# dcharatan/flowmap

Hardware: NVIDIA H100
Metric: overfit iters/sec at 150x360x640 (149 frame pairs per iteration) (higher is better)
Workload: dtype f32

## Files before the change

### flowmap_b200/csrc/fm_kernels.cu

```cuda
#include <cuda_runtime.h>
#include <stdio.h>
#include <string.h>
#include <stdlib.h>

#include "../../include/flowmap_b200.h"
#include "fm_ate.cuh"
#include "fm_host.h"
#include "fm_pixel.cuh"

namespace fm_host {
namespace {
thread_local char g_err[512] = "";
unsigned long long g_launches = 0;
}
int fail(const char* what, cudaError_t e) {
  snprintf(g_err, sizeof(g_err), "%s: %s", what, cudaGetErrorString(e));
  return 1;
}
int fail_msg(const char* what) {
  snprintf(g_err, sizeof(g_err), "%s", what);
  return 2;
}
void count_launch() { __atomic_add_fetch(&g_launches, 1, __ATOMIC_RELAXED); }
const char* last_error() { return g_err; }
// ... 1409 lines not shown
    p[i] = pp; m[i] = mm; v[i] = vv;
  }
}

__global__ void __launch_bounds__(kThreads)
k_adam_frames_ragged(float* __restrict__ p, const float* __restrict__ g, float* __restrict__ m, float* __restrict__ v,
                     size_t frame_elems, const int* __restrict__ row_offset, int pairs, int lo, int hi, float beta1,
                     float beta2, float omb1, float omb2, float eps, const float* __restrict__ consts) {
  const float step_size = __ldg(consts), bc2_sqrt = __ldg(consts + 1);
  const int span = hi - lo, b = blockIdx.y / span, f = lo + (blockIdx.y - b * span);
  const int r0 = __ldg(row_offset + b);
  if (f >= __ldg(row_offset + b + 1) - r0 - pairs) return;
  const size_t o = ((size_t)(r0 - pairs * b) + f) * frame_elems;
  p += o; g += o; m += o; v += o;
  for (size_t i = (size_t)blockIdx.x * kThreads + threadIdx.x; i < frame_elems; i += (size_t)gridDim.x * kThreads) {
    float pp = p[i], gg = g[i], mm = m[i], vv = v[i];
    FM_ADAM1(pp, gg, mm, vv)
    p[i] = pp; m[i] = mm; v[i] = vv;
  }
#undef FM_ADAM1
}

constexpr int kTrackAcc = 10;
constexpr int kTrackRec = 24;

struct SegInfo { int sample_start, rows, n, start_frame; };

struct TrackShard {
  int depth_frame0, src_lo, src_hi;
  __device__ __forceinline__ bool owns(int frame) const { return frame >= src_lo && frame < src_hi; }
};

__device__ __forceinline__ SegInfo load_seg(const int* seg, int s) {
  const int4 v = __ldg(reinterpret_cast<const int4*>(seg) + s);
  SegInfo i; i.sample_start = v.x; i.rows = v.y; i.n = v.z; i.start_frame = v.w;
  return i;
}

__device__ __forceinline__ void load_segment_frames(float* sm, const float* ext, const float* k4,
                                                    const SegInfo& si, int source_frame) {
  const float* Ps = ext + (size_t)source_frame * 16;
  for (int row = threadIdx.x; row < si.rows; row += blockDim.x) {
    const float* P = ext + (size_t)(si.start_frame + row) * 16;
    float* o = sm + row * kTrackRec;
    float v[kTrackRec];
    float* R = v;
    double t[3];
#pragma unroll
    for (int i = 0; i < 3; ++i) {
      R[i * 3 + 0] = __ldg(P + i * 4 + 0); R[i * 3 + 1] = __ldg(P + i * 4 + 1); R[i * 3 + 2] = __ldg(P + i * 4 + 2);
      t[i] = (double)__ldg(P + i * 4 + 3) - (double)__ldg(Ps + i * 4 + 3);
      v[9 + i] = (float)t[i];
    }
#pragma unroll
    for (int i = 0; i < 3; ++i)
      v[12 + i] = (float)-((double)R[0 * 3 + i] * t[0] + (double)R[1 * 3 + i] * t[1] + (double)R[2 * 3 + i] * t[2]);
    const float4 k = __ldg(reinterpret_cast<const float4*>(k4) + si.start_frame + row);
    v[15] = k.x; v[16] = k.y; v[17] = k.z; v[18] = k.w; v[19] = 1.0f / k.x; v[20] = 1.0f / k.y;
    v[21] = v[22] = v[23] = 0.f;
#pragma unroll
    for (int i = 0; i < kTrackRec / 4; ++i)
      reinterpret_cast<float4*>(o)[i] = make_float4(v[4 * i], v[4 * i + 1], v[4 * i + 2], v[4 * i + 3]);
  }
  __syncthreads();
}
static_assert(kTrackRec % 4 == 0, "frame records are read as float4");
struct TrackRec {
  float R[9], t[3], c[3];
  Cam k;
};
__device__ __forceinline__ TrackRec load_rec(const float* rec) {
  const float4* r4 = reinterpret_cast<const float4*>(rec);
  const float4 a = r4[0], b = r4[1], c = r4[2], d = r4[3], e = r4[4], f = r4[5];
  TrackRec r;
  r.R[0] = a.x; r.R[1] = a.y; r.R[2] = a.z; r.R[3] = a.w; r.R[4] = b.x; r.R[5] = b.y; r.R[6] = b.z; r.R[7] = b.w;
  r.R[8] = c.x; r.t[0] = c.y; r.t[1] = c.z; r.t[2] = c.w;
  r.c[0] = d.x; r.c[1] = d.y; r.c[2] = d.z;
  r.k.fx = d.w; r.k.fy = e.x; r.k.cx = e.y; r.k.cy = e.z; r.k.ifx = e.w; r.k.ify = f.x;
  return r;
}

struct TrackSlot { int slot; bool owner; };
template <int N, int OFF>
struct SlotWalk {
  __device__ __forceinline__ static void run(int lane, int& pos, bool& ok) {
    if (N == 1) {
      SlotWalk<1, OFF / 2>::run(lane, pos, ok);
      ok = ok && (lane & OFF) == 0;
    } else {
      constexpr int HALF = (N + 1) / 2;
      SlotWalk<HALF, OFF / 2>::run(lane, pos, ok);
      if (lane & OFF) pos += HALF;
      ok = ok && pos < N;
    }
  }
};
template <int N>
struct SlotWalk<N, 0> {
  __device__ __forceinline__ static void run(int, int& pos, bool& ok) { pos = 0; ok = true; }
};
template <int N>
__device__ __forceinline__ TrackSlot track_slot(int lane) {
  TrackSlot t;
  SlotWalk<N, 16>::run(lane, t.slot, t.owner);
  return t;
}
template <int N, int OFF>
__device__ __forceinline__ void halve_exchange(float* v, bool upper) {
  constexpr int HALF = (N + 1) / 2;
#pragma unroll
  for (int j = 0; j < HALF; ++j) {
    const float hi = (j + HALF < N) ? v[j + HALF] : 0.f;
    const float send = upper ? v[j] : hi;
    const float keep = upper ? hi : v[j];
    v[j] = keep + __shfl_xor_sync(0xffffffffu, send, OFF);
  }
}
template <int N, int OFF>
struct WarpSumN {
  __device__ __forceinline__ static void run(float* v, int lane) {
    if (N == 1) {
      v[0] += __shfl_xor_sync(0xffffffffu, v[0], OFF);
      WarpSumN<1, OFF / 2>::run(v, lane);
    } else {
      halve_exchange<N, OFF>(v, lane & OFF);
      WarpSumN<(N + 1) / 2, OFF / 2>::run(v, lane);
    }
  }
};
template <int N>
struct WarpSumN<N, 0> {
  __device__ __forceinline__ static void run(float*, int) {}
};
template <int N>
__device__ __forceinline__ float warp_sum_n(float* v, int lane) {
  WarpSumN<N, 16>::run(v, lane);
  return v[0];
}

constexpr int kTrackThreads = 128;
#ifndef FM_TRACK_PPT
#define FM_TRACK_PPT 2
#endif
#ifndef FM_TRACK_BPS
#define FM_TRACK_BPS 5
#endif
#ifndef FM_TRACK_PARTS
#define FM_TRACK_PARTS 2
#endif
constexpr int kTrackParts = FM_TRACK_PARTS;
constexpr int kTrackPPT = FM_TRACK_PPT;
constexpr int kTrackPass = 32 * kTrackPPT;
constexpr int kTrackListCap = 2048;
static_assert(kTrackPPT == 1 || kTrackPPT == 2, "FM_TRACK_PPT must be 1 or 2");

__host__ __device__ constexpr size_t track_smem_bytes(int max_rows, int list_cap) {
  return ((size_t)max_rows * (kTrackRec + (kTrackThreads / 32) * kTrackAcc) + (size_t)list_cap) * sizeof(float);
}

struct TrackOneVideo {
  static constexpr bool kPerFrameK = true;
  using Scale = Uniform::Scale;
  template <class T> __device__ __forceinline__ T* sums_of(T* sums, int) const { return sums; }
};
struct TrackVideos {
  static constexpr bool kPerFrameK = false;
  using Scale = Videos::Scale;
  const int* frame_video;
  template <class T>
  __device__ __forceinline__ T* sums_of(T* sums, int f) const { return sums + 2 * __ldg(frame_video + f); }
};

template <bool SHARED_K, class TL>
__global__ void __launch_bounds__(kTrackThreads, FM_TRACK_BPS)
k_track_src(const float* __restrict__ depth, const float* __restrict__ k4, const float* __restrict__ ext,
            const int* __restrict__ seg, const float* __restrict__ txy, const unsigned char* __restrict__ tvis,
            int mapping, float delta, double* __restrict__ sums, unsigned char* __restrict__ flag,
            float* __restrict__ dq_out, double* __restrict__ trackacc, int* __restrict__ next_item, int num_items,
            int max_rows, int list_cap, int H, int W, TrackShard sh, TL tl) {
  extern __shared__ float4 sm4[];
  __shared__ double red[kTrackAcc * (kTrackThreads / 32)];
  __shared__ int s_wbase[kTrackThreads / 32];
  __shared__ int s_item[2];
  float* sm = reinterpret_cast<float*>(sm4);
  constexpr int NW = kTrackThreads / 32;
  constexpr int NRED = SHARED_K ? 6 : kTrackAcc;
  constexpr int SLOT0 = kTrackAcc - NRED;
  float* s_tgt = sm + (size_t)max_rows * kTrackRec;
  int* s_list = reinterpret_cast<int*>(s_tgt + (size_t)NW * max_rows * kTrackAcc);
  const GridDims grid = make_grid(H, W);
  const RobustCfg rc = make_robust(mapping, delta, H, W);
  const int lane = threadIdx.x & 31, warp = threadIdx.x >> 5;
  const TrackSlot slot = track_slot<NRED>(lane);
  const float2* xy2 = reinterpret_cast<const float2*>(txy);
  for (int it = 0;; ++it) {
    if (threadIdx.x == 0) s_item[it & 1] = atomicAdd(next_item, 1);
    __syncthreads();
    const int item = s_item[it & 1];
    if (item >= num_items) break;
    const int part = item % kTrackParts, srow = item / kTrackParts;
    const SegInfo si = load_seg(seg, srow / max_rows);
    const int row = srow % max_rows;
    if (row >= si.rows || !sh.owns(si.start_frame + row)) continue;
    load_segment_frames(sm, ext, k4, si, si.start_frame + row);
    float* tgt = s_tgt + (size_t)warp * si.rows * kTrackAcc;
    for (int i = lane; i < si.rows * kTrackAcc; i += 32) tgt[i] = 0.f;
    __syncwarp();
    const int frame = si.start_frame + row;
    const float* D = depth + (size_t)(frame - sh.depth_frame0) * H * W;
    const float* rsrec = sm + row * kTrackRec;
    const size_t row0 = (size_t)si.sample_start + (size_t)row * si.n;
    const float2* seg_xy = xy2 + si.sample_start;
    const unsigned char* seg_vis = tvis + si.sample_start;
    float acc[kTrackAcc], lc[2] = {0.f, 0.f};
#pragma unroll
    for (int i = 0; i < kTrackAcc; ++i) acc[i] = 0.f;
    const int p_end = (int)((long long)si.n * (part + 1) / kTrackParts);
    for (int base = (int)((long long)si.n * part / kTrackParts); base < p_end; base += list_cap) {
      const int len = min(list_cap, p_end - base);
      const int per = (len + NW * 32 - 1) / (NW * 32) * 32;
      const int lo = base + warp * per, hi = min(base + len, lo + per);
      int cnt = 0;
      for (int p0 = lo; p0 < hi; p0 += 32) {
        const int p = p0 + lane;
        bool ok = false;
        if (p < hi) {
          const size_t sidx = row0 + p;
          const float2 sxy = __ldg(xy2 + sidx);
          ok = tvis[sidx] && in_unit_square(sxy.x, sxy.y);
          flag[sidx] = ok ? 1 : 0;
        }
        cnt += __popc(__ballot_sync(0xffffffffu, ok));
      }
      if (lane == 0) s_wbase[warp] = cnt;
      __syncthreads();
      int wb = 0, total = 0;
#pragma unroll
      for (int w = 0; w < NW; ++w) {
        const int c = s_wbase[w];
        if (w < warp) wb += c;
        total += c;
      }
      for (int p0 = lo; p0 < hi; p0 += 32) {
        const int p = p0 + lane;
        const bool ok = p < hi && flag[row0 + p];
        const unsigned m = __ballot_sync(0xffffffffu, ok);
        if (ok) s_list[wb + __popc(m & ((1u << lane) - 1u))] = p;
        wb += __popc(m);
      }
      __syncthreads();
      const int npass = (total + kTrackPass - 1) / kTrackPass;
      for (int ps = warp; ps < npass; ps += NW) {
        const int pb = ps * kTrackPass + lane;
        float Xw[kTrackPPT][3];
        int ix[kTrackPPT];
        {
          const TrackRec rs = load_rec(rsrec);
#pragma unroll
          for (int j = 0; j < kTrackPPT; ++j) {
            Xw[j][0] = Xw[j][1] = Xw[j][2] = 0.f;
            ix[j] = -1;
            if (pb + 32 * j < total) {
              const int p = s_list[pb + 32 * j];
              ix[j] = p;
              const float2 sxy = __ldg(xy2 + row0 + p);
              const Taps t = bilinear_taps(sxy.x, sxy.y, grid);
              float q[3];
              sample_surface(t, grid, rs.k, [D](int o) { return __ldg(D + o); }, q[0], q[1], q[2]);
#pragma unroll
              for (int i = 0; i < 3; ++i)
                Xw[j][i] = fm_fma(rs.R[i * 3 + 0], q[0], fm_fma(rs.R[i * 3 + 1], q[1], fm_fma(rs.R[i * 3 + 2], q[2], rs.t[i])));
            }
          }
        }
        float G[kTrackPPT][3];
#pragma unroll
        for (int j = 0; j < kTrackPPT; ++j) G[j][0] = G[j][1] = G[j][2] = 0.f;
        unsigned char vn[kTrackPPT];
        float2 gn[kTrackPPT];
#pragma unroll
        for (int j = 0; j < kTrackPPT; ++j) {
          vn[j] = ix[j] >= 0 ? seg_vis[ix[j]] : 0;
          gn[j] = ix[j] >= 0 ? __ldg(seg_xy + ix[j]) : make_float2(0.f, 0.f);
        }
        for (int ft = 0; ft < si.rows; ++ft) {
          unsigned char v[kTrackPPT];
          float2 g[kTrackPPT];
          bool any = false;
#pragma unroll
          for (int j = 0; j < kTrackPPT; ++j) {
            v[j] = vn[j]; g[j] = gn[j];
            any |= v[j] != 0;
            if (ft + 1 < si.rows && ix[j] >= 0) {
              ix[j] += si.n;
              vn[j] = seg_vis[ix[j]];
              gn[j] = __ldg(seg_xy + ix[j]);
            }
          }
          float c[NRED];
#pragma unroll
          for (int i = 0; i < NRED; ++i) c[i] = 0.f;
          bool ok = false;
          if (any) {
            const TrackRec r = load_rec(sm + ft * kTrackRec);
#pragma unroll
            for (int j = 0; j < kTrackPPT; ++j) {
              const float dir0 = fm_fma(r.R[0], Xw[j][0], fm_fma(r.R[3], Xw[j][1], __fmul_rn(r.R[6], Xw[j][2])));
              const float dir1 = fm_fma(r.R[1], Xw[j][0], fm_fma(r.R[4], Xw[j][1], __fmul_rn(r.R[7], Xw[j][2])));
              const float dir2 = fm_fma(r.R[2], Xw[j][0], fm_fma(r.R[5], Xw[j][1], __fmul_rn(r.R[8], Xw[j][2])));
              const LeanTerm lt = lean_term(1.0f, dir0, dir1, dir2, r.c[0], r.c[1], r.c[2], r.k, g[j].x, g[j].y, 0.f,
                                            0.f, 1.0f, rc);
              const bool o = v[j] && in_unit_square(lt.uvx, lt.uvy);
              ok |= o;
              const float d0 = o ? lt.d0 : 0.f, d1 = o ? lt.d1 : 0.f, d2 = o ? lt.d2 : 0.f;
              lc[0] = __fadd_rn(lc[0], o ? lt.loss : 0.f);
              lc[1] = __fadd_rn(lc[1], o ? 1.f : 0.f);
              const float g0 = fm_fma(r.R[0], d0, fm_fma(r.R[1], d1, __fmul_rn(r.R[2], d2)));
              const float g1 = fm_fma(r.R[3], d0, fm_fma(r.R[4], d1, __fmul_rn(r.R[5], d2)));
              const float g2 = fm_fma(r.R[6], d0, fm_fma(r.R[7], d1, __fmul_rn(r.R[8], d2)));
              G[j][0] = __fadd_rn(G[j][0], g0); G[j][1] = __fadd_rn(G[j][1], g1); G[j][2] = __fadd_rn(G[j][2], g2);
              const float ex = __fmul_rn(d0, r.k.ifx), ey = __fmul_rn(d1, r.k.ify);
              if (SHARED_K) {
                acc[0] = fm_fma(ex, lt.P0, acc[0]); acc[1] = fm_fma(ey, lt.P1, acc[1]);
                acc[2] = fm_fma(ex, lt.P2, acc[2]); acc[3] = fm_fma(ey, lt.P2, acc[3]);
              } else {
                c[0] = __fadd_rn(c[0], __fmul_rn(ex, lt.P0)); c[1] = __fadd_rn(c[1], __fmul_rn(ey, lt.P1));
                c[2] = __fadd_rn(c[2], __fmul_rn(ex, lt.P2)); c[3] = __fadd_rn(c[3], __fmul_rn(ey, lt.P2));
              }
              const float e0 = __fsub_rn(Xw[j][0], r.t[0]), e1 = __fsub_rn(Xw[j][1], r.t[1]);
              const float e2 = __fsub_rn(Xw[j][2], r.t[2]);
              float* tw = c + (SHARED_K ? 0 : 4);
              tw[0] = __fadd_rn(tw[0], fm_fma(e2, g1, -__fmul_rn(e1, g2)));
              tw[1] = __fadd_rn(tw[1], fm_fma(e0, g2, -__fmul_rn(e2, g0)));
              tw[2] = __fadd_rn(tw[2], fm_fma(e1, g0, -__fmul_rn(e0, g1)));
              tw[3] = __fsub_rn(tw[3], g0); tw[4] = __fsub_rn(tw[4], g1); tw[5] = __fsub_rn(tw[5], g2);
            }
          }
          if (__ballot_sync(0xffffffffu, ok)) {
            const float total_c = warp_sum_n<NRED>(c, lane);
            if (slot.owner) tgt[ft * kTrackAcc + SLOT0 + slot.slot] += total_c;
          }
        }
        const TrackRec rs = load_rec(rsrec);
#pragma unroll
        for (int j = 0; j < kTrackPPT; ++j) {
          if (pb + 32 * j >= total) continue;
          const size_t sidx = row0 + s_list[pb + 32 * j];
          const float2 sxy = __ldg(xy2 + sidx);
          const Taps t = bilinear_taps(sxy.x, sxy.y, grid);
          float q[3];
          sample_surface(t, grid, rs.k, [D](int o) { return __ldg(D + o); }, q[0], q[1], q[2]);
          const float G0 = G[j][0], G1 = G[j][1], G2 = G[j][2];
          const float dq0 = fm_fma(rs.R[0], G0, fm_fma(rs.R[3], G1, rs.R[6] * G2));
          const float dq1 = fm_fma(rs.R[1], G0, fm_fma(rs.R[4], G1, rs.R[7] * G2));
          const float dq2 = fm_fma(rs.R[2], G0, fm_fma(rs.R[5], G1, rs.R[8] * G2));
          dq_out[sidx * 3 + 0] = dq0; dq_out[sidx * 3 + 1] = dq1; dq_out[sidx * 3 + 2] = dq2;
          const float e0 = dq0 * rs.k.ifx, e1 = dq1 * rs.k.ify;
          acc[0] -= e0 * q[0]; acc[1] -= e1 * q[1]; acc[2] -= e0 * q[2]; acc[3] -= e1 * q[2];
          const float c0 = Xw[j][0] - rs.t[0], c1 = Xw[j][1] - rs.t[1], c2 = Xw[j][2] - rs.t[2];
          acc[4] += c1 * G2 - c2 * G1;
          acc[5] += c2 * G0 - c0 * G2;
          acc[6] += c0 * G1 - c1 * G0;
          acc[7] += G0; acc[8] += G1; acc[9] += G2;
        }
      }
      __syncthreads();
    }
    block_accumulate<2, kTrackThreads>(lc, tl.sums_of(sums, si.start_frame), red);
    block_accumulate<kTrackAcc, kTrackThreads>(acc, trackacc + (size_t)frame * kTrackAcc, red);
    for (int i = threadIdx.x; i < si.rows * kTrackAcc; i += kTrackThreads) {
      if (SHARED_K && i % kTrackAcc < 4) continue;
      double t = 0.0;
#pragma unroll
      for (int w = 0; w < NW; ++w) t += (double)s_tgt[(size_t)w * si.rows * kTrackAcc + i];
      if (t != 0.0) atomicAdd(trackacc + (size_t)si.start_frame * kTrackAcc + i, t);
    }
  }
}

__device__ __forceinline__ double track_scale(const double* sums, float loss_weight, const float* go) {
  double cnt = sums[1];
  if (cnt == 0.0) cnt = 1.0;
  return (double)loss_weight * (go ? (double)*go : 1.0) / cnt;
}
__device__ __forceinline__ double track_scale(const double* sums, float loss_weight, NoScale) {
  return track_scale(sums, loss_weight, nullptr);
}

__global__ void k_track_video_loss(const double* __restrict__ sums, float loss_weight, float* __restrict__ loss, int B) {
  const int b = threadIdx.x;
  if (b < B) loss[b] = (float)(track_scale(sums + 2 * b, loss_weight, nullptr) * sums[2 * b]);
}

template <class TL>
__global__ void __launch_bounds__(kThreads)
k_track_apply(const float* __restrict__ k4, const int* __restrict__ seg, const float* __restrict__ txy,
              const unsigned char* __restrict__ flag, const float* __restrict__ dq, const double* __restrict__ sums,
              float loss_weight, typename TL::Scale go, float* __restrict__ g_depth, int H, int W, TrackShard sh,
              TL tl) {
  const SegInfo si = load_seg(seg, blockIdx.z);
  const int row = blockIdx.y;
  const int p = blockIdx.x * kThreads + threadIdx.x;
  if (row >= si.rows || p >= si.n || !sh.owns(si.start_frame + row)) return;
  const size_t sidx = (size_t)si.sample_start + (size_t)row * si.n + p;
  if (!flag[sidx]) return;
  const float scale = (float)track_scale(tl.sums_of(sums, si.start_frame), loss_weight, go);
  const int frame = si.start_frame + row;
  const GridDims grid = make_grid(H, W);
  const Cam ks = make_cam(load_k4(k4, frame));
  const float2 sxy = __ldg(reinterpret_cast<const float2*>(txy) + sidx);
  const Taps t = bilinear_taps(sxy.x, sxy.y, grid);
  const float dq0 = scale * dq[sidx * 3 + 0], dq1 = scale * dq[sidx * 3 + 1], dq2 = scale * dq[sidx * 3 + 2];
  float rx0, ry0, rx1, ry1;
  tap_rays(t, grid, ks, rx0, ry0, rx1, ry1);
  float* gd = g_depth + (size_t)(frame - sh.depth_frame0) * H * W;
  red_add(gd + t.y0 * W + t.x0, t.w00 * (dq0 * rx0 + dq1 * ry0 + dq2));
  red_add(gd + t.y0 * W + t.x1, t.w01 * (dq0 * rx1 + dq1 * ry0 + dq2));
  red_add(gd + t.y1 * W + t.x0, t.w10 * (dq0 * rx0 + dq1 * ry1 + dq2));
  red_add(gd + t.y1 * W + t.x1, t.w11 * (dq0 * rx1 + dq1 * ry1 + dq2));
}

template <class TL>
__global__ void k_track_finalize(const double* __restrict__ trackacc, const double* __restrict__ sums,
                                 float loss_weight, typename TL::Scale go, const float* __restrict__ ext,
                                 float* __restrict__ g_ext, float* __restrict__ g_k4, int F, TL tl) {
  const int f = blockIdx.x * blockDim.x + threadIdx.x;
  if (f >= F) return;
  const double sc = track_scale(tl.sums_of(sums, f), loss_weight, go);
  const double* a = trackacc + (size_t)f * kTrackAcc;
  for (int k = 0; k < 4; ++k) g_k4[(size_t)f * 4 + k] = (float)(sc * a[k]);
  const float* P = ext + (size_t)f * 16;
  const double w0 = 0.5 * sc * a[4], w1 = 0.5 * sc * a[5], w2 = 0.5 * sc * a[6];
  float* o = g_ext + (size_t)f * 16;
  for (int c = 0; c < 3; ++c) {
    const double r0 = P[0 * 4 + c], r1 = P[1 * 4 + c], r2 = P[2 * 4 + c];
    o[0 * 4 + c] = (float)(-w2 * r1 + w1 * r2);
    o[1 * 4 + c] = (float)(w2 * r0 - w0 * r2);
    o[2 * 4 + c] = (float)(-w1 * r0 + w0 * r1);
  }
  o[3] = (float)(sc * a[7]); o[7] = (float)(sc * a[8]); o[11] = (float)(sc * a[9]);
  o[12] = o[13] = o[14] = o[15] = 0.f;
}

constexpr int kSweepAcc = 80;

__global__ void k_sweep_base_k4(const float* __restrict__ cand_k4, float* __restrict__ base_k4, int B, int n) {
  const int t = blockIdx.x * blockDim.x + threadIdx.x;
  if (t >= B * 8) return;
  const int b = t >> 3, e = t & 7;
  base_k4[t] = cand_k4[(size_t)b * n * 8 + e];
}

__global__ void k_sweep_scale_solve(const double* __restrict__ base_moments, const float* __restrict__ base_zshift,
                                    const float* __restrict__ cand_k4, float* __restrict__ rt,
                                    PairState* __restrict__ state, int B, int n) {
  const int item = blockIdx.x * blockDim.x + threadIdx.x;
  if (item >= B * n) return;
  const int b = item / n;
  const double z0 = (double)base_zshift[b];
  const double sx = (double)cand_k4[(size_t)b * n * 8 + 0] / (double)cand_k4[(size_t)item * 8 + 0];
  const double sy = (double)cand_k4[(size_t)b * n * 8 + 1] / (double)cand_k4[(size_t)item * 8 + 1];
  const double sc[3] = {sx, sy, 1.0};
  double m[kNumMoments];
  const double* bm = base_moments + (size_t)b * kNumMoments;
  m[0] = bm[0];
  for (int i = 0; i < 3; ++i) { m[1 + i] = bm[1 + i] * sc[i]; m[4 + i] = bm[4 + i] * sc[i]; }
  for (int a = 0; a < 3; ++a)
    for (int c = 0; c < 3; ++c) m[7 + a * 3 + c] = bm[7 + a * 3 + c] * sc[a] * sc[c];
  const double shift[3] = {0.0, 0.0, z0};
  PairState st;
  float out[12];
  procrustes_solve(m, shift, out, st);
  for (int k = 0; k < 12; ++k) rt[(size_t)item * 12 + k] = out[k];
  state[item] = st;
}

__global__ void k_sweep_aggregate(const PairAdjoint* __restrict__ adj, const float* __restrict__ cand_k4,
                                  PairAdjoint* __restrict__ out, int B, int n) {
  const int b = blockIdx.x, lane = threadIdx.x;
  double acc[16];
#pragma unroll
  for (int i = 0; i < 16; ++i) acc[i] = 0.0;
  for (int c = lane; c < n; c += 32) {
    const int item = b * n + c;
    const PairAdjoint a = adj[item];
    const double s[3] = {(double)cand_k4[(size_t)b * n * 8 + 0] / (double)cand_k4[(size_t)item * 8 + 0],
                         (double)cand_k4[(size_t)b * n * 8 + 1] / (double)cand_k4[(size_t)item * 8 + 1], 1.0};
#pragma unroll
    for (int r = 0; r < 3; ++r) {
      double cq = 0.0, cp = 0.0;
#pragma unroll
      for (int k = 0; k < 3; ++k) {
        acc[r * 3 + k] += s[r] * (double)a.cbar[r * 3 + k] * s[k];
        cq += (double)a.cbar[k * 3 + r] * (double)a.qbar[k];
        cp += (double)a.cbar[r * 3 + k] * (double)a.pbar[k];
      }
      acc[9 + r] += s[r] * ((double)a.pb[r] - cq);
      acc[12 + r] += s[r] * ((double)a.qb[r] - cp);
      acc[15] += (double)a.qbar[r] * cp - (double)a.pb[r] * (double)a.pbar[r] - (double)a.qb[r] * (double)a.qbar[r];
    }
  }
#pragma unroll
  for (int i = 0; i < 16; ++i) acc[i] = warp_sum(acc[i]);
  if (lane == 0) {
    PairAdjoint o;
    for (int i = 0; i < 9; ++i) o.cbar[i] = (float)acc[i];
    for (int i = 0; i < 3; ++i) {
      o.pb[i] = (float)acc[9 + i]; o.qb[i] = (float)acc[12 + i]; o.pbar[i] = 0.f; o.qbar[i] = 0.f;
      o.shift[i] = adj[b * n].shift[i];
    }
    o.wconst = (float)acc[15];
    out[b] = o;
  }
}

template <bool BWD, class Lay>
__global__ void __launch_bounds__(kThreads)
k_sweep(const float* __restrict__ depth, const float* __restrict__ k4, const float* __restrict__ rt,
        const float* __restrict__ bflow, const float* __restrict__ weights, float wsens,
        const int64_t* __restrict__ indices, int num_indices, const float* __restrict__ g_err,
        double* __restrict__ acc_out, float* __restrict__ g_depth, float* __restrict__ g_weights, Lay lay, int H,
        int W) {
  __shared__ double smem[12 * (kThreads / 32)];
  const int item = blockIdx.y;
  const int N = H * W;
  const PairAddr pa = pair_addr(lay, item, N);
  const Cam ka = make_cam(load_k4(k4, pa.k4_frame_a));
  const Cam kb = make_cam(load_k4(k4, pa.k4_frame_a + 1));
// ... 1026 lines not shown
  k_pose_chain<<<B, kChainThreads, 0, (cudaStream_t)stream>>>(rt, extrinsics, lay);
  FM_CHECK_LAUNCH("fm_pose_chain");
  return 0;
}
template <class Lay>
static int pose_chain_bwd(const float* rt, const float* extrinsics, const float* g_extrinsics, float* g_rt, int B,
                          const Lay& lay, void* stream) {
  k_pose_chain_bwd<<<B, kChainThreads, 0, (cudaStream_t)stream>>>(rt, extrinsics, g_extrinsics, g_rt, lay);
  FM_CHECK_LAUNCH("fm_pose_chain_bwd");
  return 0;
}

}

int fm_pose_chain(const float* rt, float* extrinsics, int B, int F, void* stream) {
  if (!rt || !extrinsics || B < 1 || F < 2) return fail_msg("fm_pose_chain: bad arguments");
  return pose_chain(rt, extrinsics, B, Uniform{F}, stream);
}

int fm_trajectory_ate(const float* gt, const float* pred, int T, int F, float* ate, float* aligned_gt,
                      float* aligned_pred, int* status, void* stream) {
  if (!gt || !pred || !ate || !status || T < 0 || F < 1) return fail_msg("fm_trajectory_ate: bad arguments");
  if (T == 0) return 0;
  MetricsRow none;
  memset(&none, 0, sizeof(none));
  k_trajectory_ate<<<T, kAteThreads, 0, (cudaStream_t)stream>>>(gt, pred, 3, 1, F, ate, aligned_gt, aligned_pred,
                                                                status, none);
  FM_CHECK_LAUNCH("fm_trajectory_ate");
  return 0;
}

int fm_pose_chain_bwd(const float* rt, const float* extrinsics, const float* g_extrinsics, float* g_rt,
                      int B, int F, void* stream) {
  if (!rt || !extrinsics || !g_extrinsics || !g_rt || B < 1 || F < 2) return fail_msg("fm_pose_chain_bwd: bad arguments");
  return pose_chain_bwd(rt, extrinsics, g_extrinsics, g_rt, B, Uniform{F}, stream);
}

int fm_step_clock_tick(void* clock, double lr, double beta1, double beta2, unsigned long long base_seed,
                       int tick_focal, void* stream) {
  if (!clock) return fail_msg("fm_step_clock_tick: bad arguments");
  k_clock_tick<<<1, 1, 0, (cudaStream_t)stream>>>((StepClock*)clock, lr, beta1, beta2, base_seed, tick_focal);
  FM_CHECK_LAUNCH("fm_step_clock_tick");
  return 0;
}

int fm_adam_step_clock(float* param, const float* grad, float* exp_avg, float* exp_avg_sq, size_t count,
                       const void* clock, int focal_clock, double beta1_d, double beta2_d, double eps_d,
                       void* stream) {
  if (!param || !grad || !exp_avg || !exp_avg_sq || !clock) return fail_msg("fm_adam_step_clock: bad arguments");
  if (count == 0) return 0;
  size_t nb = (count / 4 + kThreads * 2 - 1) / (kThreads * 2);
  if (nb < 1) nb = 1;
  if (nb > (size_t)sm_count_cached() * 16) nb = (size_t)sm_count_cached() * 16;
  const StepClock* c = (const StepClock*)clock;
  k_adam<<<(unsigned)nb, kThreads, 0, (cudaStream_t)stream>>>(
      param, grad, exp_avg, exp_avg_sq, count, (float)beta1_d, (float)beta2_d, (float)(1.0 - beta1_d),
      (float)(1.0 - beta2_d), (float)eps_d, 0.f, 1.f, focal_clock ? &c->focal_step_size : &c->step_size);
  FM_CHECK_LAUNCH("fm_adam_step_clock");
  return 0;
}

int fm_random_subset_clock(const void* clock, long long N, int n, int64_t* out, void* stream) {
  if (!clock || N < 1 || n < 1 || n > N || !out) return fail_msg("fm_random_subset_clock: bad arguments");
  k_random_subset<<<(n + 127) / 128, 128, 0, (cudaStream_t)stream>>>(0ull, N, n, out, &((const StepClock*)clock)->seed);
  FM_CHECK_LAUNCH("fm_random_subset_clock");
  return 0;
}

int fm_adam_step(float* param, const float* grad, float* exp_avg, float* exp_avg_sq, size_t count,
                 double lr, double beta1_d, double beta2_d, double eps_d, int step, void* stream) {
  if (!param || !grad || !exp_avg || !exp_avg_sq || step < 1) return fail_msg("fm_adam_step: bad arguments");
  if (count == 0) return 0;
  const float beta1 = (float)beta1_d, beta2 = (float)beta2_d, eps = (float)eps_d;
  const double bc1 = 1.0 - pow(beta1_d, (double)step);
  const double bc2 = 1.0 - pow(beta2_d, (double)step);
  const float step_size = (float)(lr / bc1);
  const float bc2_sqrt = (float)sqrt(bc2);
  size_t nb = (count / 4 + kThreads * 2 - 1) / (kThreads * 2);
  if (nb < 1) nb = 1;
  if (nb > (size_t)sm_count_cached() * 16) nb = (size_t)sm_count_cached() * 16;
  k_adam<<<(unsigned)nb, kThreads, 0, (cudaStream_t)stream>>>(param, grad, exp_avg, exp_avg_sq, count, beta1, beta2, (float)(1.0 - (double)beta1_d), (float)(1.0 - (double)beta2_d), eps, step_size, bc2_sqrt);
  FM_CHECK_LAUNCH("fm_adam_step");
  return 0;
}

size_t fm_track_workspace_bytes(int F, long long total_samples) {
  if (F < 1 || total_samples < 0) return 0;
  size_t off = 0;
  off = align_up(off + 4 * sizeof(double), 256);
  off = align_up(off + (size_t)F * kTrackAcc * sizeof(double), 256);
  off = align_up(off + (size_t)total_samples * 3 * sizeof(float), 256);
  off = align_up(off + (size_t)total_samples, 256);
  return off;
}

namespace {
struct TrackWs { double* sums; int* next_item; double* acc; float* dq; unsigned char* flag; };
TrackWs carve_track(void* base, int F, long long total) {
  char* p = (char*)base; size_t off = 0; TrackWs w;
  w.sums = (double*)(p + off); w.next_item = (int*)(p + off + 4 * sizeof(double));
  off = align_up(off + 4 * sizeof(double), 256);
  w.acc = (double*)(p + off); off = align_up(off + (size_t)F * kTrackAcc * sizeof(double), 256);
  w.dq = (float*)(p + off); off = align_up(off + (size_t)total * 3 * sizeof(float), 256);
  w.flag = (unsigned char*)(p + off);
  return w;
}
}

size_t fm_track_reduce_bytes(int F) {
  if (F < 1) return 0;
  return align_up(4 * sizeof(double), 256) + align_up((size_t)F * kTrackAcc * sizeof(double), 256);
}

extern "C++" {
template <class TL>
static int track_fwd_impl(const float* depth, const float* k4, const float* extrinsics, const int* segments,
                          int num_segments, int max_rows, int max_points, const float* track_xy,
                          const unsigned char* track_vis, long long total_samples, int mapping, float delta,
                          float loss_weight, float* loss, void* ws, int F, int H, int W, int depth_frame0,
                          int src_frame_lo, int src_frame_hi, int shared_intrinsics, void* stream, double* sums,
                          int B, const TL& tl) {
  if (!depth || !k4 || !extrinsics || !segments || !track_xy || !track_vis || !ws ||
      num_segments < 1 || max_rows < 1 || max_points < 1 || F < 1)
    return fail_msg("fm_track_loss_fwd: bad arguments");
  if (mapping < 0 || mapping > 2) return fail_msg("fm_track_loss_fwd: unknown mapping");
  if (depth_frame0 < 0 || src_frame_lo < depth_frame0 || src_frame_hi > F || src_frame_lo > src_frame_hi)
    return fail_msg("fm_track_loss_fwd: bad source-frame range");
  cudaStream_t s = (cudaStream_t)stream;
  TrackWs w = carve_track(ws, F, total_samples);
  cudaError_t e = cudaMemsetAsync(w.sums, 0, (char*)w.dq - (char*)w.sums, s);
  if (e != cudaSuccess) return fail("fm_track_loss_fwd: memset", e);
  if (sums != w.sums && (e = cudaMemsetAsync(sums, 0, (size_t)B * 2 * sizeof(double), s)) != cudaSuccess)
    return fail("fm_track_loss_fwd: memset", e);
  const int list_cap = max_points < kTrackListCap ? max_points : kTrackListCap;
  const size_t smem = track_smem_bytes(max_rows, list_cap);
  if (smem > 200 * 1024) return fail_msg("fm_track_loss_fwd: segment too long for shared memory");
  const long long items = (long long)num_segments * max_rows * kTrackParts;
  if (items > INT_MAX) return fail_msg("fm_track_loss_fwd: too many segment rows");
  int per_sm = (int)((227 * 1024) / (smem + sizeof(double) * kTrackAcc * (kTrackThreads / 32) + 1024 + 64));
  if (per_sm > FM_TRACK_BPS) per_sm = FM_TRACK_BPS;
  if (per_sm < 1) per_sm = 1;
  const int grid = persistent_grid(per_sm, items);
  auto src = k_track_src<true, TL>;
  if constexpr (TL::kPerFrameK) {
    if (!shared_intrinsics) src = k_track_src<false, TL>;
  } else if (!shared_intrinsics) {
    return fail_msg("fm_track_loss_fwd: packed videos have one focal length each");
  }
  if (smem > 48 * 1024) {
    const cudaError_t ea = cudaFuncSetAttribute(src, cudaFuncAttributeMaxDynamicSharedMemorySize, (int)smem);
    if (ea != cudaSuccess) return fail("fm_track_loss_fwd: shared memory", ea);
  }
  const TrackShard sh = {depth_frame0, src_frame_lo, src_frame_hi};
  src<<<grid, kTrackThreads, smem, s>>>(depth, k4, extrinsics, segments, track_xy, track_vis, mapping, delta, sums,
                                        w.flag, w.dq, w.acc, w.next_item, (int)items, max_rows, list_cap, H, W, sh, tl);
  FM_CHECK_LAUNCH("fm_track_loss_fwd: k_track_src");
  if (loss) {
    k_track_video_loss<<<1, 32 * ((B + 31) / 32), 0, s>>>(sums, loss_weight, loss, B);
    FM_CHECK_LAUNCH("fm_track_loss_fwd: k_track_video_loss");
  }
  return 0;
}

}

int fm_track_loss_fwd_sharded(const float* depth, const float* k4, const float* extrinsics, const int* segments,
                              int num_segments, int max_rows, int max_points, const float* track_xy,
                              const unsigned char* track_vis, long long total_samples, int mapping, float delta,
                              float loss_weight, float* loss, void* ws, int F, int H, int W, int depth_frame0,
                              int src_frame_lo, int src_frame_hi, int shared_intrinsics, void* stream) {
  return track_fwd_impl(depth, k4, extrinsics, segments, num_segments, max_rows, max_points, track_xy, track_vis,
                        total_samples, mapping, delta, loss_weight, loss, ws, F, H, W, depth_frame0, src_frame_lo,
                        src_frame_hi, shared_intrinsics, stream, (double*)ws, 1, TrackOneVideo{});
}

int fm_track_loss_fwd(const float* depth, const float* k4, const float* extrinsics, const int* segments,
                      int num_segments, int max_rows, int max_points, const float* track_xy,
                      const unsigned char* track_vis, long long total_samples, int mapping, float delta,
                      float loss_weight, float* loss, void* ws, int F, int H, int W, void* stream) {
  if (!loss) return fail_msg("fm_track_loss_fwd: bad arguments");
  return fm_track_loss_fwd_sharded(depth, k4, extrinsics, segments, num_segments, max_rows, max_points, track_xy,
                                   track_vis, total_samples, mapping, delta, loss_weight, loss, ws, F, H, W, 0,
                                   0, F, 0, stream);
}

int fm_track_loss_value(const void* ws, float loss_weight, float* loss, void* stream) {
  if (!ws || !loss) return fail_msg("fm_track_loss_value: bad arguments");
  k_track_video_loss<<<1, 32, 0, (cudaStream_t)stream>>>((const double*)ws, loss_weight, loss, 1);
  FM_CHECK_LAUNCH("fm_track_loss_value");
  return 0;
}

extern "C++" {
template <class TL>
static int track_bwd_impl(const float* k4, const float* extrinsics, const int* segments, int num_segments,
                          int max_rows, int max_points, const float* track_xy, long long total_samples,
                          float loss_weight, const float* grad_out, float* g_depth, float* g_extrinsics,
                          float* g_k4, void* ws, int F, int H, int W, int depth_frame0, int src_frame_lo,
                          int src_frame_hi, cudaStream_t s, cudaStream_t apply_stream, const double* sums,
                          const TL& tl) {
  if (!k4 || !extrinsics || !segments || !track_xy || !g_depth || !g_extrinsics || !g_k4 || !ws ||
      num_segments < 1 || max_rows < 1 || max_points < 1 || F < 1)
    return fail_msg("fm_track_loss_bwd: bad arguments");
  if (depth_frame0 < 0 || src_frame_lo < depth_frame0 || src_frame_hi > F || src_frame_lo > src_frame_hi)
    return fail_msg("fm_track_loss_bwd: bad source-frame range");
  TrackWs w = carve_track(ws, F, total_samples);
  dim3 grid((max_points + kThreads - 1) / kThreads, max_rows, num_segments);
  const TrackShard sh = {depth_frame0, src_frame_lo, src_frame_hi};
  k_track_apply<TL><<<grid, kThreads, 0, apply_stream>>>(k4, segments, track_xy, w.flag, w.dq, sums, loss_weight,
                                                        grad_out, g_depth, H, W, sh, tl);
  FM_CHECK_LAUNCH("fm_track_loss_bwd: k_track_apply");
  k_track_finalize<TL><<<(F + 63) / 64, 64, 0, s>>>(w.acc, sums, loss_weight, grad_out, extrinsics, g_extrinsics,
                                                   g_k4, F, tl);
  FM_CHECK_LAUNCH("fm_track_loss_bwd: k_track_finalize");
  return 0;
}

}

int fm_track_loss_bwd_sharded(const float* depth, const float* k4, const float* extrinsics, const int* segments,
                              int num_segments, int max_rows, int max_points, const float* track_xy,
                              const unsigned char* track_vis, long long total_samples, int mapping, float delta,
                              float loss_weight, const float* grad_out, float* g_depth, float* g_extrinsics,
                              float* g_k4, void* ws, int F, int H, int W, int depth_frame0, int src_frame_lo,
                              int src_frame_hi, void* stream) {
  (void)depth; (void)track_vis; (void)mapping; (void)delta;
  return track_bwd_impl(k4, extrinsics, segments, num_segments, max_rows, max_points, track_xy, total_samples,
                        loss_weight, grad_out, g_depth, g_extrinsics, g_k4, ws, F, H, W, depth_frame0,
                        src_frame_lo, src_frame_hi, (cudaStream_t)stream, (cudaStream_t)stream, (const double*)ws,
                        TrackOneVideo{});
}

int fm_track_loss_bwd(const float* depth, const float* k4, const float* extrinsics, const int* segments,
                      int num_segments, int max_rows, int max_points, const float* track_xy,
                      const unsigned char* track_vis, long long total_samples, int mapping, float delta,
                      float loss_weight, const float* grad_out, float* g_depth, float* g_extrinsics,
                      float* g_k4, void* ws, int F, int H, int W, void* stream) {
  return fm_track_loss_bwd_sharded(depth, k4, extrinsics, segments, num_segments, max_rows, max_points, track_xy,
                                   track_vis, total_samples, mapping, delta, loss_weight, grad_out, g_depth,
                                   g_extrinsics, g_k4, ws, F, H, W, 0, 0, F, stream);
}

size_t fm_points_workspace_bytes(int items) {
  if (items < 1) return 0;
  return carve(nullptr, items, 2).bytes;
}

int fm_align_rigid_fwd(const float* p, const float* q, const float* weights, float* rt, void* ws, int items,
                       int n, void* stream) {
  if (!p || !q || !weights || !rt || !ws || items < 1 || n < 1) return fail_msg("fm_align_rigid_fwd: bad arguments");
  cudaStream_t s = (cudaStream_t)stream;
  Workspace w = carve(ws, items, 2);
  cudaError_t e = cudaMemsetAsync(w.moments, 0, (size_t)items * kNumMoments * sizeof(double), s);
  if (e != cudaSuccess) return fail("fm_align_rigid_fwd: memset", e);
  k_points_shift<<<items, kThreads, 0, s>>>(p, q, weights, w.pshift, n);
  FM_CHECK_LAUNCH("fm_align_rigid_fwd: k_points_shift");
  dim3 grid(blocks_for(n, 1), items);
  k_points_moments<<<grid, kThreads, 0, s>>>(p, q, weights, w.pshift, w.moments, n);
  FM_CHECK_LAUNCH("fm_align_rigid_fwd: k_points_moments");
  k_points_solve<<<(items + 63) / 64, 64, 0, s>>>(w.moments, w.pshift, rt, w.state, items);
  FM_CHECK_LAUNCH("fm_align_rigid_fwd: k_points_solve");
  return 0;
}

int fm_align_rigid_bwd(const float* p, const float* q, const float* weights, const float* g_rt, float* g_p,
                       float* g_q, float* g_w, void* ws, int items, int n, void* stream) {
  if (!p || !q || !weights || !g_rt || !g_p || !g_q || !g_w || !ws || items < 1 || n < 1)
    return fail_msg("fm_align_rigid_bwd: bad arguments");
  cudaStream_t s = (cudaStream_t)stream;
  Workspace w = carve(ws, items, 2);
  k_adjoint<<<(items + 63) / 64, 64, 0, s>>>(w.flowacc, w.state, g_rt, 0, nullptr, w.adj, items, Uniform{2});
  FM_CHECK_LAUNCH("fm_align_rigid_bwd: k_adjoint");
  dim3 grid(blocks_for(n, 1), items);
  k_points_distribute<<<grid, kThreads, 0, s>>>(p, q, weights, w.adj, g_p, g_q, g_w, n);
  FM_CHECK_LAUNCH("fm_align_rigid_bwd: k_points_distribute");
  return 0;
}

int fm_unproject_points(const float* xy, const float* z, const float* k4, float* out, int items, int n,
                        int xy_shared, void* stream) {
  if (!xy || !z || !k4 || !out || items < 1 || n < 1) return fail_msg("fm_unproject_points: bad arguments");
  dim3 grid(blocks_for(n, 1), items);
  k_unproject_points<<<grid, kThreads, 0, (cudaStream_t)stream>>>(xy, z, k4, out, n, xy_shared);
  FM_CHECK_LAUNCH("fm_unproject_points");
  return 0;
}

int fm_unproject_points_bwd(const float* xy, const float* z, const float* k4, const float* g_out, float* g_z,
                            float* g_k4, void* ws, int items, int n, int xy_shared, void* stream) {
  if (!xy || !z || !k4 || !g_out || !g_z || !g_k4 || !ws || items < 1 || n < 1)
    return fail_msg("fm_unproject_points_bwd: bad arguments");
  cudaStream_t s = (cudaStream_t)stream;
  Workspace w = carve(ws, items, 2);
  cudaError_t e = cudaMemsetAsync(w.k4acc, 0, (size_t)items * 4 * sizeof(double), s);
  if (e != cudaSuccess) return fail("fm_unproject_points_bwd: memset", e);
  dim3 grid(blocks_for(n, 1), items);
  k_unproject_points_bwd<<<grid, kThreads, 0, s>>>(xy, z, k4, g_out, g_z, w.k4acc, n, xy_shared);
  FM_CHECK_LAUNCH("fm_unproject_points_bwd: k_unproject_points_bwd");
  k_d2f<<<(items * 4 + 127) / 128, 128, 0, s>>>(w.k4acc, g_k4, items * 4);
  FM_CHECK_LAUNCH("fm_unproject_points_bwd: k_d2f");
  return 0;
}

int fm_random_subset(unsigned long long seed, long long N, int n, int64_t* out, void* stream) {
  if (!out || N < 1 || n < 1 || n > N || N > (1ll << 40)) return fail_msg("fm_random_subset: bad arguments");
  k_random_subset<<<(n + 127) / 128, 128, 0, (cudaStream_t)stream>>>(seed, N, n, out);
  FM_CHECK_LAUNCH("fm_random_subset");
  return 0;
// ... 349 lines not shown
```

Before: 391.4.

## Streamline track loss inner loop with precomputed robust params and deferred rotation

Moves the robust-loss config to the host and passes a precomputed TrackRobust struct, so the fast path in the per-frame track loop becomes branch-light: a specialized track_tail runs when all lanes have finite projections and falls back to lean_term otherwise. The per-target accumulators now store gradients in camera space, and the rotation by the target frame's R is deferred to a per-frame double-precision epilogue. This removes the per-point world-space rotation and subtraction from the hot loop. Visibility becomes a bitmask that keeps the loads unconditional, and the 'any' early-skip is dropped, so every frame is now computed. The changed rounding order may perturb results slightly.

```diff
diff --git a/flowmap_b200/csrc/fm_kernels.cu b/flowmap_b200/csrc/fm_kernels.cu
--- a/flowmap_b200/csrc/fm_kernels.cu
+++ b/flowmap_b200/csrc/fm_kernels.cu
@@ -1585,7 +1585,43 @@
 constexpr int kTrackPPT = FM_TRACK_PPT;
 constexpr int kTrackPass = 32 * kTrackPPT;
 constexpr int kTrackListCap = 2048;
-static_assert(kTrackPPT == 1 || kTrackPPT == 2, "FM_TRACK_PPT must be 1 or 2");
+static_assert(kTrackPPT >= 1 && kTrackPPT <= 4, "FM_TRACK_PPT must be 1 to 4");
+
+struct TrackRobust {
+  float ax, ay, thr, qk, qv, off;
+  bool l2;
+};
+FM_HD TrackRobust make_track_robust(const RobustCfg& rc) {
+  TrackRobust t;
+  const bool huber = rc.mapping == MAP_HUBER;
+  t.ax = rc.ax;
+  t.ay = rc.ay;
+  t.l2 = rc.mapping == MAP_L2;
+  t.thr = huber ? rc.delta : -1.0f;
+  t.qk = t.l2 ? 1.0f : rc.inv_delta;
+  t.qv = t.l2 ? 0.5f : 0.5f * rc.inv_delta;
+  t.off = huber ? 0.5f * rc.delta : 0.0f;
+  return t;
+}
+__device__ __forceinline__ void track_tail(LeanTerm& t, float u0, float u1, float u2, float inv, const Cam& k,
+                                           float x, float y, const TrackRobust& rb) {
+  const float uvx = fm_fma(k.fx, u0, k.cx * u2), uvy = fm_fma(k.fy, u1, k.cy * u2);
+  t.uvx = uvx;
+  t.uvy = uvy;
+  const float sx = (uvx - x) * rb.ax, sy = (uvy - y) * rb.ay;
+  const float n2 = fm_fma(sx, sx, sy * sy);
+  const float inv_n = n2 > kTinyNorm2 ? fm_rsqrt(n2) : 0.0f;
+  const float n = n2 * inv_n;
+  const bool quad = rb.l2 || n <= rb.thr;
+  const float kk = quad ? rb.qk : inv_n;
+  t.loss = quad ? rb.qv * n2 : n - rb.off;
+  const float duvx = sx * (kk * rb.ax), duvy = sy * (kk * rb.ay);
+  const float du0 = k.fx * duvx, du1 = k.fy * duvy, du2 = fm_fma(k.cx, duvx, k.cy * duvy);
+  t.d0 = du0 * inv;
+  t.d1 = du1 * inv;
+  const float dot = fm_fma(du0, t.P0, fm_fma(du1, t.P1, du2 * t.P2));
+  t.d2 = fm_fma(-dot, inv, du2) * inv;
+}
 
 __host__ __device__ constexpr size_t track_smem_bytes(int max_rows, int list_cap) {
   return ((size_t)max_rows * (kTrackRec + (kTrackThreads / 32) * kTrackAcc) + (size_t)list_cap) * sizeof(float);
@@ -1608,7 +1644,7 @@
 __global__ void __launch_bounds__(kTrackThreads, FM_TRACK_BPS)
 k_track_src(const float* __restrict__ depth, const float* __restrict__ k4, const float* __restrict__ ext,
             const int* __restrict__ seg, const float* __restrict__ txy, const unsigned char* __restrict__ tvis,
-            int mapping, float delta, double* __restrict__ sums, unsigned char* __restrict__ flag,
+            RobustCfg rc, TrackRobust rb, double* __restrict__ sums, unsigned char* __restrict__ flag,
             float* __restrict__ dq_out, double* __restrict__ trackacc, int* __restrict__ next_item, int num_items,
             int max_rows, int list_cap, int H, int W, TrackShard sh, TL tl) {
   extern __shared__ float4 sm4[];
@@ -1622,7 +1658,6 @@
   float* s_tgt = sm + (size_t)max_rows * kTrackRec;
   int* s_list = reinterpret_cast<int*>(s_tgt + (size_t)NW * max_rows * kTrackAcc);
   const GridDims grid = make_grid(H, W);
-  const RobustCfg rc = make_robust(mapping, delta, H, W);
   const int lane = threadIdx.x & 31, warp = threadIdx.x >> 5;
   const TrackSlot slot = track_slot<NRED>(lane);
   const float2* xy2 = reinterpret_cast<const float2*>(txy);
@@ -1686,16 +1721,18 @@
       for (int ps = warp; ps < npass; ps += NW) {
         const int pb = ps * kTrackPass + lane;
         float Xw[kTrackPPT][3];
-        int ix[kTrackPPT];
+        unsigned ix[kTrackPPT];
+        unsigned live = 0;
         {
           const TrackRec rs = load_rec(rsrec);
 #pragma unroll
           for (int j = 0; j < kTrackPPT; ++j) {
             Xw[j][0] = Xw[j][1] = Xw[j][2] = 0.f;
-            ix[j] = -1;
+            ix[j] = 0;
             if (pb + 32 * j < total) {
               const int p = s_list[pb + 32 * j];
               ix[j] = p;
+              live |= 1u << j;
               const float2 sxy = __ldg(xy2 + row0 + p);
               const Taps t = bilinear_taps(sxy.x, sxy.y, grid);
               float q[3];
@@ -1709,65 +1746,81 @@
         float G[kTrackPPT][3];
 #pragma unroll
         for (int j = 0; j < kTrackPPT; ++j) G[j][0] = G[j][1] = G[j][2] = 0.f;
-        unsigned char vn[kTrackPPT];
+        unsigned vn[kTrackPPT];
         float2 gn[kTrackPPT];
 #pragma unroll
         for (int j = 0; j < kTrackPPT; ++j) {
-          vn[j] = ix[j] >= 0 ? seg_vis[ix[j]] : 0;
-          gn[j] = ix[j] >= 0 ? __ldg(seg_xy + ix[j]) : make_float2(0.f, 0.f);
+          vn[j] = seg_vis[ix[j]];
+          gn[j] = __ldg(seg_xy + ix[j]);
         }
         for (int ft = 0; ft < si.rows; ++ft) {
-          unsigned char v[kTrackPPT];
+          bool v[kTrackPPT];
           float2 g[kTrackPPT];
-          bool any = false;
 #pragma unroll
           for (int j = 0; j < kTrackPPT; ++j) {
-            v[j] = vn[j]; g[j] = gn[j];
-            any |= v[j] != 0;
-            if (ft + 1 < si.rows && ix[j] >= 0) {
-              ix[j] += si.n;
+            v[j] = ((live >> j) & 1u) && vn[j] != 0u;
+            g[j] = gn[j];
+          }
+          if (ft + 1 < si.rows) {
+#pragma unroll
+            for (int j = 0; j < kTrackPPT; ++j) {
+              ix[j] += (unsigned)si.n;
               vn[j] = seg_vis[ix[j]];
               gn[j] = __ldg(seg_xy + ix[j]);
             }
           }
+          const TrackRec r = load_rec(sm + ft * kTrackRec);
+          LeanTerm lt[kTrackPPT];
+          float u[kTrackPPT][3], inv[kTrackPPT];
+          bool fin = true;
+#pragma unroll
+          for (int j = 0; j < kTrackPPT; ++j) {
+            lt[j].P0 = fm_fma(r.R[0], Xw[j][0], fm_fma(r.R[3], Xw[j][1], fm_fma(r.R[6], Xw[j][2], r.c[0])));
+            lt[j].P1 = fm_fma(r.R[1], Xw[j][0], fm_fma(r.R[4], Xw[j][1], fm_fma(r.R[7], Xw[j][2], r.c[1])));
+            lt[j].P2 = fm_fma(r.R[2], Xw[j][0], fm_fma(r.R[5], Xw[j][1], fm_fma(r.R[8], Xw[j][2], r.c[2])));
+            inv[j] = fm_rcp(lt[j].P2 + kProjEps);
+            u[j][0] = lt[j].P0 * inv[j]; u[j][1] = lt[j].P1 * inv[j]; u[j][2] = lt[j].P2 * inv[j];
+            fin = fin && (fabsf(u[j][0]) + fabsf(u[j][1])) + fabsf(u[j][2]) <= 3.0e38f;
+          }
+          if (__all_sync(0xffffffffu, fin)) {
+#pragma unroll
+            for (int j = 0; j < kTrackPPT; ++j)
+              track_tail(lt[j], u[j][0], u[j][1], u[j][2], inv[j], r.k, g[j].x, g[j].y, rb);
+          } else {
+#pragma unroll
+            for (int j = 0; j < kTrackPPT; ++j)
+              lt[j] = lean_term(1.0f, lt[j].P0, lt[j].P1, lt[j].P2, 0.f, 0.f, 0.f, r.k, g[j].x, g[j].y, 0.f, 0.f,
+                                1.0f, rc);
+          }
           float c[NRED];
 #pragma unroll
           for (int i = 0; i < NRED; ++i) c[i] = 0.f;
           bool ok = false;
-          if (any) {
-            const TrackRec r = load_rec(sm + ft * kTrackRec);
-#pragma unroll
-            for (int j = 0; j < kTrackPPT; ++j) {
-              const float dir0 = fm_fma(r.R[0], Xw[j][0], fm_fma(r.R[3], Xw[j][1], __fmul_rn(r.R[6], Xw[j][2])));
-              const float dir1 = fm_fma(r.R[1], Xw[j][0], fm_fma(r.R[4], Xw[j][1], __fmul_rn(r.R[7], Xw[j][2])));
-              const float dir2 = fm_fma(r.R[2], Xw[j][0], fm_fma(r.R[5], Xw[j][1], __fmul_rn(r.R[8], Xw[j][2])));
-              const LeanTerm lt = lean_term(1.0f, dir0, dir1, dir2, r.c[0], r.c[1], r.c[2], r.k, g[j].x, g[j].y, 0.f,
-                                            0.f, 1.0f, rc);
-              const bool o = v[j] && in_unit_square(lt.uvx, lt.uvy);
-              ok |= o;
-              const float d0 = o ? lt.d0 : 0.f, d1 = o ? lt.d1 : 0.f, d2 = o ? lt.d2 : 0.f;
-              lc[0] = __fadd_rn(lc[0], o ? lt.loss : 0.f);
-              lc[1] = __fadd_rn(lc[1], o ? 1.f : 0.f);
-              const float g0 = fm_fma(r.R[0], d0, fm_fma(r.R[1], d1, __fmul_rn(r.R[2], d2)));
-              const float g1 = fm_fma(r.R[3], d0, fm_fma(r.R[4], d1, __fmul_rn(r.R[5], d2)));
-              const float g2 = fm_fma(r.R[6], d0, fm_fma(r.R[7], d1, __fmul_rn(r.R[8], d2)));
-              G[j][0] = __fadd_rn(G[j][0], g0); G[j][1] = __fadd_rn(G[j][1], g1); G[j][2] = __fadd_rn(G[j][2], g2);
-              const float ex = __fmul_rn(d0, r.k.ifx), ey = __fmul_rn(d1, r.k.ify);
-              if (SHARED_K) {
-                acc[0] = fm_fma(ex, lt.P0, acc[0]); acc[1] = fm_fma(ey, lt.P1, acc[1]);
-                acc[2] = fm_fma(ex, lt.P2, acc[2]); acc[3] = fm_fma(ey, lt.P2, acc[3]);
-              } else {
-                c[0] = __fadd_rn(c[0], __fmul_rn(ex, lt.P0)); c[1] = __fadd_rn(c[1], __fmul_rn(ey, lt.P1));
-                c[2] = __fadd_rn(c[2], __fmul_rn(ex, lt.P2)); c[3] = __fadd_rn(c[3], __fmul_rn(ey, lt.P2));
-              }
-              const float e0 = __fsub_rn(Xw[j][0], r.t[0]), e1 = __fsub_rn(Xw[j][1], r.t[1]);
-              const float e2 = __fsub_rn(Xw[j][2], r.t[2]);
-              float* tw = c + (SHARED_K ? 0 : 4);
-              tw[0] = __fadd_rn(tw[0], fm_fma(e2, g1, -__fmul_rn(e1, g2)));
-              tw[1] = __fadd_rn(tw[1], fm_fma(e0, g2, -__fmul_rn(e2, g0)));
-              tw[2] = __fadd_rn(tw[2], fm_fma(e1, g0, -__fmul_rn(e0, g1)));
-              tw[3] = __fsub_rn(tw[3], g0); tw[4] = __fsub_rn(tw[4], g1); tw[5] = __fsub_rn(tw[5], g2);
+#pragma unroll
+          for (int j = 0; j < kTrackPPT; ++j) {
+            const bool o = v[j] && in_unit_square(lt[j].uvx, lt[j].uvy);
+            ok |= o;
+            const float d0 = o ? lt[j].d0 : 0.f, d1 = o ? lt[j].d1 : 0.f, d2 = o ? lt[j].d2 : 0.f;
+            if (o) {
+              lc[0] = __fadd_rn(lc[0], lt[j].loss);
+              lc[1] = __fadd_rn(lc[1], 1.f);
             }
+            G[j][0] = __fadd_rn(G[j][0], fm_fma(r.R[0], d0, fm_fma(r.R[1], d1, __fmul_rn(r.R[2], d2))));
+            G[j][1] = __fadd_rn(G[j][1], fm_fma(r.R[3], d0, fm_fma(r.R[4], d1, __fmul_rn(r.R[5], d2))));
+            G[j][2] = __fadd_rn(G[j][2], fm_fma(r.R[6], d0, fm_fma(r.R[7], d1, __fmul_rn(r.R[8], d2))));
+            const float ex = __fmul_rn(d0, r.k.ifx), ey = __fmul_rn(d1, r.k.ify);
+            if (SHARED_K) {
+              acc[0] = fm_fma(ex, lt[j].P0, acc[0]); acc[1] = fm_fma(ey, lt[j].P1, acc[1]);
+              acc[2] = fm_fma(ex, lt[j].P2, acc[2]); acc[3] = fm_fma(ey, lt[j].P2, acc[3]);
+            } else {
+              c[0] = __fadd_rn(c[0], __fmul_rn(ex, lt[j].P0)); c[1] = __fadd_rn(c[1], __fmul_rn(ey, lt[j].P1));
+              c[2] = __fadd_rn(c[2], __fmul_rn(ex, lt[j].P2)); c[3] = __fadd_rn(c[3], __fmul_rn(ey, lt[j].P2));
+            }
+            float* tw = c + (SHARED_K ? 0 : 4);
+            tw[0] = __fadd_rn(tw[0], fm_fma(d1, lt[j].P2, -__fmul_rn(d2, lt[j].P1)));
+            tw[1] = __fadd_rn(tw[1], fm_fma(d2, lt[j].P0, -__fmul_rn(d0, lt[j].P2)));
+            tw[2] = __fadd_rn(tw[2], fm_fma(d0, lt[j].P1, -__fmul_rn(d1, lt[j].P0)));
+            tw[3] = __fadd_rn(tw[3], d0); tw[4] = __fadd_rn(tw[4], d1); tw[5] = __fadd_rn(tw[5], d2);
           }
           if (__ballot_sync(0xffffffffu, ok)) {
             const float total_c = warp_sum_n<NRED>(c, lane);
@@ -1801,12 +1854,28 @@
     }
     block_accumulate<2, kTrackThreads>(lc, tl.sums_of(sums, si.start_frame), red);
     block_accumulate<kTrackAcc, kTrackThreads>(acc, trackacc + (size_t)frame * kTrackAcc, red);
-    for (int i = threadIdx.x; i < si.rows * kTrackAcc; i += kTrackThreads) {
-      if (SHARED_K && i % kTrackAcc < 4) continue;
-      double t = 0.0;
-#pragma unroll
-      for (int w = 0; w < NW; ++w) t += (double)s_tgt[(size_t)w * si.rows * kTrackAcc + i];
-      if (t != 0.0) atomicAdd(trackacc + (size_t)si.start_frame * kTrackAcc + i, t);
+    for (int ft = threadIdx.x; ft < si.rows; ft += kTrackThreads) {
+      double t[kTrackAcc];
+#pragma unroll
+      for (int i = SLOT0; i < kTrackAcc; ++i) {
+        t[i] = 0.0;
+#pragma unroll
+        for (int w = 0; w < NW; ++w) t[i] += (double)s_tgt[((size_t)w * si.rows + ft) * kTrackAcc + i];
+      }
+      const float* R = sm + ft * kTrackRec;
+      double o[kTrackAcc];
+#pragma unroll
+      for (int i = SLOT0; i < 4; ++i) o[i] = t[i];
+#pragma unroll
+      for (int i = 0; i < 3; ++i) {
+        const double r0 = R[i * 3 + 0], r1 = R[i * 3 + 1], r2 = R[i * 3 + 2];
+        o[4 + i] = r0 * t[4] + r1 * t[5] + r2 * t[6];
+        o[7 + i] = -(r0 * t[7] + r1 * t[8] + r2 * t[9]);
+      }
+      double* dst = trackacc + (size_t)(si.start_frame + ft) * kTrackAcc;
+#pragma unroll
+      for (int i = SLOT0; i < kTrackAcc; ++i)
+        if (o[i] != 0.0) atomicAdd(dst + i, o[i]);
     }
   }
 }
@@ -3139,8 +3208,10 @@
     if (ea != cudaSuccess) return fail("fm_track_loss_fwd: shared memory", ea);
   }
   const TrackShard sh = {depth_frame0, src_frame_lo, src_frame_hi};
-  src<<<grid, kTrackThreads, smem, s>>>(depth, k4, extrinsics, segments, track_xy, track_vis, mapping, delta, sums,
-                                        w.flag, w.dq, w.acc, w.next_item, (int)items, max_rows, list_cap, H, W, sh, tl);
+  const RobustCfg rc = make_robust(mapping, delta, H, W);
+  src<<<grid, kTrackThreads, smem, s>>>(depth, k4, extrinsics, segments, track_xy, track_vis, rc,
+                                        make_track_robust(rc), sums, w.flag, w.dq, w.acc, w.next_item, (int)items,
+                                        max_rows, list_cap, H, W, sh, tl);
   FM_CHECK_LAUNCH("fm_track_loss_fwd: k_track_src");
   if (loss) {
     k_track_video_loss<<<1, 32 * ((B + 31) / 32), 0, s>>>(sums, loss_weight, loss, B);
```

Result: faster. 401.2, median of 6 (+2.5%).
